# alexbuburuzan/MObI

Hardware: AMD Instinct MI355X
Metric: denoising throughput (UNet element-forwards/s = steps/s x UNet batch) (higher is better)
Workload: dtype bf16; 1 GPU; mobi_nusc_512 UNet denoising step, 8 objects/GPU (UNet batch 16), latent 64x64, DDIM-50 schedule, cfg_scale 1.0; objects_per_gpu=8, unet_batch=16, latent=64, sampler=ddim, parallelism=dp1 (objects sharded, no collective in the loop)

## Files before the change

### mobi_amd/csrc/igemm.hip

```cpp
#include <stdlib.h>

#include <type_traits>

#include "common.h"
#include "tuning.h"
#include "igemm_small.h"

#ifndef MOBI_FRAG2
#define MOBI_FRAG2 0
#endif
#ifndef MOBI_DMA_KS
#define MOBI_DMA_KS 1
#endif
#if defined(MOBI_IGEMM_FENCE) && MOBI_IGEMM_FENCE
#define MOBI_SCHED_FENCE() __builtin_amdgcn_sched_barrier(0)
#else
#define MOBI_SCHED_FENCE() ((void)0)
#endif

#ifndef MOBI_DBG_SKIP
#define MOBI_DBG_SKIP 0
#endif
#ifndef MOBI_PP_DMA_KS
#define MOBI_PP_DMA_KS 1
// ... 2515 lines not shown
    dim3 block(512);
    dim3 pgrid(grid.x < (unsigned)compute_units() ? grid.x : (unsigned)compute_units(), grid.y, grid.z);
    if (a.split_ws) {
      if (nt5) hipLaunchKernelGGL((igemm_pp_kernel<T, 5, false, true>), pgrid, block, 0, st, a);
      else     hipLaunchKernelGGL((igemm_pp_kernel<T, 4, false, true>), pgrid, block, 0, st, a);
    } else {
#define MOBI_PP_LAUNCH(NT_, G_) hipLaunchKernelGGL((igemm_pp_kernel<T, NT_, G_>), pgrid, block, 0, st, a)
      if (a.epilogue == MOBI_EPI_GEGLU) { if (nt5) MOBI_PP_LAUNCH(5, true); else MOBI_PP_LAUNCH(4, true); }
      else                              { if (nt5) MOBI_PP_LAUNCH(5, false); else MOBI_PP_LAUNCH(4, false); }
#undef MOBI_PP_LAUNCH
    }
  }
#ifdef MOBI_DEV
  else if (a.wm == 4 && a.fast && a.glds) {
    dim3 block(512);
    dim3 pgrid(grid.x < (unsigned)compute_units() ? grid.x : (unsigned)compute_units(), grid.y, grid.z);
    const int mode = tr ? 1 : (a.epi_direct ? (a.epilogue == MOBI_EPI_GEGLU ? 3 : 2) : 0);
#define MOBI_GLDS_LAUNCH(NT_, MODE_) hipLaunchKernelGGL((igemm_glds_kernel<T, NT_, MODE_>), pgrid, block, 0, st, a)
#define MOBI_GLDS_BY_MODE(NT_)                                                                     \
  do { switch (mode) { case 0: MOBI_GLDS_LAUNCH(NT_, 0); break; case 1: MOBI_GLDS_LAUNCH(NT_, 1); break; \
                       case 2: MOBI_GLDS_LAUNCH(NT_, 2); break; default: MOBI_GLDS_LAUNCH(NT_, 3); break; } } while (0)
    if (nt5) MOBI_GLDS_BY_MODE(5); else MOBI_GLDS_BY_MODE(4);
#undef MOBI_GLDS_BY_MODE
#undef MOBI_GLDS_LAUNCH
  }
#endif
  else if (a.wm == 4) { if (nt5) MOBI_IGEMM_BY_TR(5, 4); else MOBI_IGEMM_BY_TR(4, 4); }
  else if (a.sm && a.sm64) {
#define MOBI_SM64_LAUNCH_W(NT_, TR_, LNF_, OVL_) \
  hipLaunchKernelGGL((igemm_ring64_kernel<T, NT_, TR_, LNF_, OVL_>), grid, dim3(256), 0, st, a)
#define MOBI_SM64_LAUNCH(NT_, TR_, LNF_) \
  do { if (tuning().sm64_ovl != 0) MOBI_SM64_LAUNCH_W(NT_, TR_, LNF_, true); else MOBI_SM64_LAUNCH_W(NT_, TR_, LNF_, false); } while (0)
    if (a.ln_svec) { if (nt5) MOBI_SM64_LAUNCH(5, false, true); else MOBI_SM64_LAUNCH(4, false, true); }
    else if (nt5) { if (tr) MOBI_SM64_LAUNCH(5, true, false); else MOBI_SM64_LAUNCH(5, false, false); }
    else     { if (tr) MOBI_SM64_LAUNCH(4, true, false); else MOBI_SM64_LAUNCH(4, false, false); }
#undef MOBI_SM64_LAUNCH
#undef MOBI_SM64_LAUNCH_W
  }
  else if (a.sm) {
#define MOBI_SM_LAUNCH(NT_, TR_) hipLaunchKernelGGL((igemm_ring_kernel<T, NT_, TR_, 4, 4>), grid, dim3(256), 0, st, a)
    if (a.ln_svec) {
      if (nt5) hipLaunchKernelGGL((igemm_ring_kernel<T, 5, false, 4, 4, true>), grid, dim3(256), 0, st, a);
      else     hipLaunchKernelGGL((igemm_ring_kernel<T, 4, false, 4, 4, true>), grid, dim3(256), 0, st, a);
    }
    else if (nt5) { if (tr) MOBI_SM_LAUNCH(5, true); else MOBI_SM_LAUNCH(5, false); }
    else     { if (tr) MOBI_SM_LAUNCH(4, true); else MOBI_SM_LAUNCH(4, false); }
#undef MOBI_SM_LAUNCH
  }
  else                { if (nt5) MOBI_IGEMM_BY_TR(5, 2); else MOBI_IGEMM_BY_TR(4, 2); }
#undef MOBI_IGEMM_BY_TR
#undef MOBI_IGEMM_BY_FAST
#undef MOBI_IGEMM_LAUNCH
  MOBI_CHECK_LAUNCH();
  if (a.split_ws && !a.sync && !p->defer_finish) return launch_splitk_reduce<T>(a, st);
  return MOBI_OK;
}

constexpr int SMALL_MFLOP_DEFAULT = 1800, SMALL_MFLOP_K320 = 1000, SMALL_CONV_M_DEFAULT = 0;
static int small_tile(const mobi_igemm_params* p) {
  if (tuning().small == 0) return 0;
  if (tuning().small < 0 && (tuning().wm == 2 || tuning().wm == 4 || tuning().wide >= 0 || tuning().sm == 0)) return 0;
  const bool conv3 = p->kh == 3 && p->kw == 3 && p->pad_h == 1 && p->pad_w == 1;
  if (!(p->kh == 1 && p->kw == 1) && !conv3) return 0;
  if (p->stride != 1 || p->upsample || p->groups != 1 || p->epilogue != MOBI_EPI_NONE || p->k_order != 0 || p->split_k > 1) return 0;
  if (p->out_mode != MOBI_OUT_ROWS && p->out_mode != MOBI_OUT_ROWS_F32) return 0;
  if (p->hout != p->hin || p->wout != p->win) return 0;
  const int ct = p->c0 + p->c1, N = p->n_packed;
  const long long K = (long long)ct * p->kh * p->kw;
  if (ct % 320 || (p->c1 > 0 && p->c0 % 80) || N != p->cout || N % 32) return 0;
  const long long hw = (long long)p->hin * p->win, M = (long long)p->batch * hw;
  const long long ips = p->src_img_stride ? p->src_img_stride / p->c0 : hw;
  const long long cmax = p->c0 > p->c1 ? p->c0 : p->c1;
  if ((((long long)p->batch - 1) * ips + hw) * cmax * 2 >= 0x7fffffffLL || (long long)N * K * 2 >= 0x7fffffffLL) return 0;
  if (tuning().small > 0) return 32;
  if (conv3) {
    const int cap_m = tuning().small_conv_m >= 0 ? tuning().small_conv_m : SMALL_CONV_M_DEFAULT;
    return M <= cap_m ? 32 : 0;
  }
  const int cap = tuning().small_mflop >= 0 ? tuning().small_mflop : (K == 320 ? SMALL_MFLOP_K320 : SMALL_MFLOP_DEFAULT);
  if (2.0 * (double)M * N * (double)K > 1e6 * cap) return 0;
  return 32;
}

static int plan_splits(long long M, int n_packed, int ktot) {
  const int bn = (n_packed % 160) == 0 ? 160 : 128;
  const long long tiles = ((M + 127) / 128) * ((n_packed + bn - 1) / bn);
  const int nk = (ktot + 63) / 64;
  const bool r5 = tuning().split_round4 != 0;
  if (tiles >= 384 || nk < (r5 ? 24 : 16)) return 1;
  if (tiles >= 256 && (r5 ? nk <= 40 : nk < 40)) return 1;
  const long long target = tuning().split_target > 0 ? tuning().split_target : 512;
  long long s = (target + tiles - 1) / tiles;
  const long long cap = tiles <= 16 ? 16 : 8;
  if (s > cap) s = cap;
  if (s > nk / 8) s = nk / 8;
  if (r5) {
    if (s > 4 && s < 8) s = 4;
    if (s == 8 && nk <= 96 && tiles >= 64) s = 4;
  }
  if (tiles >= 128 && tiles <= 256 && s >= 2 && nk / s >= 80 && tuning().split_longk != 0) s *= 2;
  return s < 2 ? 1 : (int)s;
}

}

#if MOBI_STAMP
extern "C" int mobi_debug_set_stamps(void* buf) {
  return hipMemcpyToSymbol(HIP_SYMBOL(mobi::g_stamps), &buf, sizeof(void*)) == hipSuccess ? MOBI_OK : MOBI_ERR_LAUNCH;
}
#endif
#if MOBI_STAMP >= 2
extern "C" int mobi_debug_set_phases(void* buf) {
  return hipMemcpyToSymbol(HIP_SYMBOL(mobi::g_phase), &buf, sizeof(void*)) == hipSuccess ? MOBI_OK : MOBI_ERR_LAUNCH;
}
#endif

extern "C" int mobi_igemm_plan_splits(const mobi_igemm_params* p) {
  if (!p || p->groups != 1 || p->epilogue != MOBI_EPI_NONE || p->out_mode == MOBI_OUT_TRANSPOSED || p->ln_svec) return 1;
  {
    mobi_igemm_params q = *p;
    q.split_k = 0;
    if (mobi::small_tile(&q)) return 1;
  }
  return mobi::plan_splits((long long)p->batch * p->hout * p->wout, p->n_packed, p->kh * p->kw * (p->c0 + p->c1));
}

extern "C" size_t mobi_igemm_workspace_bytes(const mobi_igemm_params* p, int32_t splits) {
  if (!p || splits <= 1) return 0;
  return (size_t)splits * p->batch * p->hout * p->wout * p->n_packed * sizeof(float);
}

extern "C" size_t mobi_igemm_sync_bytes(const mobi_igemm_params* p, int32_t splits) {
  if (!p || splits <= 1) return 0;
  const size_t m = (size_t)p->batch * p->hout * p->wout;
  return ((m + 127) / 128) * (((size_t)p->n_packed + 127) / 128) * sizeof(int32_t);
}

static int igemm_prepare(const mobi_igemm_params* p, mobi::IgemmArgs& a) {
  using namespace mobi;
  if (!p || !p->src0 || !p->weight || !p->out) return MOBI_ERR_ARG;
  if (p->dtype != MOBI_F16 && p->dtype != MOBI_BF16) return MOBI_ERR_ARG;
  if (p->c0 <= 0 || (p->c0 & 31) || p->c1 < 0 || (p->c1 & 31) || (p->c1 > 0 && !p->src1)) return MOBI_ERR_UNSUPPORTED;
  if (p->batch <= 0 || p->hin <= 0 || p->win <= 0 || p->hout <= 0 || p->wout <= 0) return MOBI_ERR_ARG;
  if (p->kh <= 0 || p->kw <= 0 || p->stride <= 0 || p->groups <= 0 || p->batch % p->groups) return MOBI_ERR_ARG;
  if (p->cout <= 0 || p->n_packed <= 0) return MOBI_ERR_ARG;
  if (p->upsample != 0 && p->upsample != 1) return MOBI_ERR_ARG;
  const bool geglu = p->epilogue == MOBI_EPI_GEGLU;
  const bool leaky = p->epilogue == MOBI_EPI_LEAKY_RELU;
  if (p->epilogue != MOBI_EPI_NONE && !geglu && !leaky) return MOBI_ERR_ARG;
  if (leaky && (p->out_mode == MOBI_OUT_TRANSPOSED || p->ln_svec || p->split_k > 1 || p->k_order != 0))
    return MOBI_ERR_UNSUPPORTED;
  if (p->out_mode < 0 || p->out_mode > 2) return MOBI_ERR_ARG;
  if (p->out_mode != MOBI_OUT_TRANSPOSED && (p->cout & 7)) return MOBI_ERR_UNSUPPORTED;
  if (geglu && (p->out_mode != MOBI_OUT_ROWS || p->rowvec || p->residual)) return MOBI_ERR_UNSUPPORTED;
  if (!geglu && p->n_packed != p->cout) return MOBI_ERR_ARG;
  if (geglu && p->n_packed != 2 * p->cout) return MOBI_ERR_ARG;
  if (p->out_mode == MOBI_OUT_TRANSPOSED && (p->rowvec || p->residual)) return MOBI_ERR_UNSUPPORTED;
  if ((reinterpret_cast<uintptr_t>(p->bias) | reinterpret_cast<uintptr_t>(p->rowvec)) & 15) return MOBI_ERR_ALIGN;
  if (p->rowvec && (p->rowvec_stride & 3)) return MOBI_ERR_ALIGN;
  if ((reinterpret_cast<uintptr_t>(p->src0) | reinterpret_cast<uintptr_t>(p->src1) |
       reinterpret_cast<uintptr_t>(p->weight) | reinterpret_cast<uintptr_t>(p->out) |
       reinterpret_cast<uintptr_t>(p->residual)) & 15) return MOBI_ERR_ALIGN;

  const bool lnf = p->ln_svec != nullptr;
  if (lnf) {
    if (p->kh != 1 || p->kw != 1 || p->c1 || p->stride != 1 || p->upsample || p->groups != 1 || p->split_k > 1 || p->rowvec ||
        p->residual || p->out_mode == MOBI_OUT_TRANSPOSED || p->scale != 1.0f || p->k_order != 0 || p->hout != p->hin || p->wout != p->win)
      return MOBI_ERR_UNSUPPORTED;
    if (reinterpret_cast<uintptr_t>(p->ln_svec) & 15) return MOBI_ERR_ALIGN;
  }
  a.ln_svec = p->ln_svec; a.ln_eps = p->ln_eps;
  a.src0 = p->src0; a.src1 = p->src1;
  a.c0 = p->c0; a.c1 = p->c1; a.C = p->c0 + p->c1;
  a.hin = p->hin; a.win = p->win; a.up = p->upsample;
  a.hout = p->hout; a.wout = p->wout; a.hw_out = p->hout * p->wout;
  a.kh = p->kh; a.kw = p->kw; a.stride = p->stride; a.pad_h = p->pad_h; a.pad_w = p->pad_w;
  const long long hw_in = (long long)p->hin * p->win;
  if (p->src_img_stride && (p->c1 || p->src_img_stride % p->c0)) return MOBI_ERR_UNSUPPORTED;
  const long long ips = p->src_img_stride ? p->src_img_stride / p->c0 : hw_in;
  if (ips * p->batch > 0x7fffffffLL) return MOBI_ERR_UNSUPPORTED;
  a.img_pix_stride = (int)ips;
  a.weight = p->weight; a.w_group_stride = p->groups > 1 ? p->w_group_stride : 0;
  a.n_packed = p->n_packed; a.cout = p->cout;
  a.ktot = p->kh * p->kw * a.C;
  a.nk = (a.ktot + 63) / 64;
  a.imgs_per_group = p->batch / p->groups;
  a.M = a.imgs_per_group * a.hw_out;
  a.bias = p->bias; a.rowvec = p->rowvec; a.residual = p->residual;
  a.rowvec_stride = p->rowvec_stride ? p->rowvec_stride : p->cout;
  a.res_img_stride = p->res_img_stride ? p->res_img_stride : (long long)a.hw_out * p->cout;
  a.out = p->out;
  a.out_img_stride = p->out_img_stride ? p->out_img_stride : (long long)a.hw_out * p->cout;
  a.out_mode = p->out_mode; a.epilogue = p->epilogue; a.scale = p->scale;
  const int bn = (p->n_packed % 160) == 0 ? 160 : 128;
  {
    const long long tiles256 = ((a.M + 255) / 256) * (long long)((p->n_packed + bn - 1) / bn);
    a.wm = tiles256 >= 256 ? 4 : 2;
    if (p->split_k > 1 && a.M % 256 == 0 && tiles256 * p->split_k >= 256 && a.nk / p->split_k >= 16) a.wm = 4;
    if (tuning().pp_split == 0 && p->split_k > 1 && tiles256 < 256) a.wm = 2;
    if (tuning().wm == 2 || tuning().wm == 4) a.wm = tuning().wm;
  }
  a.tiles_m = (a.M + 64 * a.wm - 1) / (64 * a.wm);
  bool ring_ok = false;
  {
    const long long ext0 = (((long long)p->batch - 1) * ips + hw_in) * p->c0 * 2;
    const long long ext1 = p->c1 ? (((long long)p->batch - 1) * ips + hw_in) * p->c1 * 2 : 0;
    const long long wext = (long long)p->n_packed * a.ktot * 2;
// ... 185 lines not shown
```

### mobi_amd/ldm/modules/attention.py

```python
import os
import weakref

import torch
import torch.nn as nn

from ... import engine_dtype, ops
from ..._lib import ACT_NONE
from .diffusionmodules.util import Conv2d, GroupNorm32, LayerNorm, Linear, Marker, enter, leave, zero_module


FUSED_FF = os.environ.get("MOBI_FUSED_FF", "1") != "0"
FUSED_FF_MIN_ROWS = int(os.environ.get("MOBI_FUSED_FF_MIN_ROWS", "24576"))
FUSED_LN = os.environ.get("MOBI_FUSED_LN", "1") != "0"
ROW_CHAIN = os.environ.get("MOBI_ROW_CHAIN", "1") != "0"
LN_FOLD = os.environ.get("MOBI_LN_FOLD", "1") != "0"
LN_FOLD_MIN_ROWS = int(os.environ.get("MOBI_LN_FOLD_MIN_ROWS", "512"))
GROUPED_Q = os.environ.get("MOBI_GROUPED_Q", "1") != "0"
ROW_CHAIN_MIN_ROWS = int(os.environ.get("MOBI_ROW_CHAIN_MIN_ROWS", "24576"))
PRE_CHAIN = os.environ.get("MOBI_PRE_CHAIN", "0") == "1"


def _store_in_place(old, new):
    if isinstance(new, torch.Tensor):
        if isinstance(old, torch.Tensor) and old.shape == new.shape and old.dtype == new.dtype \
                and old.device == new.device and old.is_contiguous() and old.data_ptr() != new.data_ptr():
            old.copy_(new)
            return old
        return new.contiguous()
    if isinstance(new, tuple):
        if not (isinstance(old, tuple) and len(old) == len(new)):
            old = (None,) * len(new)
        return tuple(_store_in_place(o, n) for o, n in zip(old, new))
    return new


def Normalize(in_channels):
    return GroupNorm32(32, in_channels, eps=1e-6)


class GEGLU(nn.Module):
    def __init__(self, dim_in, dim_out):
        super().__init__()
        self.proj = Linear(dim_in, dim_out * 2)

    def forward(self, x, ln=None):
        if ln is None:
            return ops.linear(x, self.proj.packed_geglu())
        ps = (self.proj.weight, self.proj.bias, ln.weight, ln.bias)
        key = tuple(p._version for p in ps) + (ps[0].data_ptr(), ps[0].device, engine_dtype(), ln.eps)
        c = self.__dict__.setdefault("_ln_cache", {})
        if c.get("key") != key:
            w, b = ops.fold_layernorm(self.proj.weight, self.proj.bias, ln.weight, ln.bias)
            c["key"], c["val"] = key, ops.with_row_sums(ops.pack_geglu(w, b, engine_dtype(), self.proj.weight.device), ln.eps)
        return ops.linear(x, c["val"])


class FeedForward(nn.Module):
    def __init__(self, dim, dim_out=None, mult=4, glu=False, dropout=0.):
        super().__init__()
        if not glu:
            raise NotImplementedError("MObI's transformer blocks use gated_ff=True")
        inner_dim = int(dim * mult)
        dim_out = dim if dim_out is None else dim_out
        self.net = nn.Sequential(GEGLU(dim, inner_dim), Marker(), Linear(inner_dim, dim_out))

    def _fused(self):
        proj, out = self.net[0].proj, self.net[2]
        c, hidden = out.weight.shape
        if not (FUSED_FF and ops.ff_geglu_supported(c, hidden) and proj.weight.shape == (2 * hidden, c)):
            return None
        ps = (proj.weight, proj.bias, out.weight, out.bias)
        key = tuple(p._version for p in ps) + (ps[0].data_ptr(), ps[0].device, engine_dtype())
        cache = self.__dict__.setdefault("_fused_cache", {})
        if cache.get("key") != key:
            cache["key"], cache["val"] = key, ops.pack_ff_geglu(proj.weight, proj.bias, out.weight, out.bias, engine_dtype(),
                                                                proj.weight.device)
        return cache["val"]

    def forward(self, x, residual=None, norm=None):
        rows = x.numel() // x.shape[-1]
        pf = self._fused() if (rows >= FUSED_FF_MIN_ROWS and x.is_contiguous()
                               and (residual is None or residual.is_contiguous())) else None
        if pf is not None:
            if norm is not None and FUSED_LN:
                return ops.ff_geglu(x, pf, residual=residual, ln=(*norm.affine(), norm.eps))
            if norm is not None:
                x = ops.layernorm(x, *norm.affine(), norm.eps)
            return ops.ff_geglu(x, pf, residual=residual)
        if norm is not None and LN_FOLD and x.is_contiguous() and rows >= LN_FOLD_MIN_ROWS:
            return ops.linear(self.net[0](x, ln=norm), self.net[2].packed(), residual=residual)
        if norm is not None:
            x = ops.layernorm(x, *norm.affine(), norm.eps)
        return ops.linear(self.net[0](x), self.net[2].packed(), residual=residual)


class CrossAttention(nn.Module):
    def __init__(self, query_dim, context_dim=None, heads=8, dim_head=64, dropout=0.):
        super().__init__()
        inner_dim = dim_head * heads
        context_dim = query_dim if context_dim is None else context_dim
        self.scale = dim_head ** -0.5
        self.heads = heads
        self.inner_dim = inner_dim
        self.to_q = Linear(query_dim, inner_dim, bias=False)
        self.to_k = Linear(context_dim, inner_dim, bias=False)
        self.to_v = Linear(context_dim, inner_dim, bias=False)
        self.to_out = nn.Sequential(Linear(inner_dim, query_dim), Marker())

    def _stacked(self, names, fold_q=False, ln=None):
        mods = [getattr(self, n) for n in names]
        dtype = engine_dtype()
        key = (names, fold_q, dtype, self.scale) + tuple(v for m in mods for v in (m.weight._version, m.weight.data_ptr()))
        if ln is not None:
            key += (ln.weight._version, ln.bias._version, ln.weight.data_ptr(), ln.eps)
        c = self.__dict__.setdefault("_stack_cache", {})
        slot = (names, fold_q, ln is not None)
        hit = c.get(slot)
        if hit is None or hit[0] != key:
            ws = [m.weight.detach() for m in mods]
            if fold_q:
                assert names[0] == "to_q"
                ws[0] = ws[0].float() * (self.scale * ops.LOG2E)
            w = torch.cat([w_.float() for w_ in ws], dim=0) if (fold_q or ln is not None) else torch.cat(ws, dim=0)
            if ln is not None:
                wf, bf = ops.fold_layernorm(w, None, ln.weight, ln.bias)
                hit = (key, ops.with_row_sums(ops.pack_linear(wf, bf, dtype, w.device), ln.eps))
            else:
                hit = (key, ops.pack_linear(w, None, dtype, w.device))
            c[slot] = hit
        return hit[1]

    def self_attention(self, xn, ln=None):
        c = self.inner_dim
        qkv = ops.linear(xn, self._stacked(("to_q", "to_k", "to_v"), fold_q=True, ln=ln))
        return ops.attention(qkv[..., :c], qkv[..., c:2 * c], qkv[..., 2 * c:], self.heads, self.scale, v_rows=True,
                             q_log2_scaled=True)

    def token_attention(self, xn, ctx, q=None):
        c = self.inner_dim
        if q is not None:
            kv = ops.linear(ctx, self._stacked(("to_k", "to_v")))
        else:
            q, kv = ops.concurrently(lambda: ops.linear(xn, self._stacked(("to_q",), fold_q=True)),
                                     lambda: ops.linear(ctx, self._stacked(("to_k", "to_v"))))
        return ops.attention(q, kv[..., :c], kv[..., c:], self.heads, self.scale, v_rows=True, q_log2_scaled=True)

    def context_kv(self, context):
        n, tk, cc = context.shape
        flat = context.reshape(n * tk, cc)
        wk, _ = self.to_k.skinny()
        wv, _ = self.to_v.skinny()
        k = ops.skinny_linear(flat, wk).reshape(n, tk, self.inner_dim)
        v = ops.skinny_linear(flat, wv).reshape(n, tk, self.inner_dim)
        return k, v

    def few_token_attention(self, xn, context):
        q, (k, v) = ops.concurrently(lambda: ops.linear(xn, self.to_q.packed()), lambda: self.context_kv(context))
        return ops.ctx_attention(q, k, v, self.heads, self.scale)

    def single_token_vector(self, token, extra_bias=None):
        wv, _ = self.to_v.skinny()
        wo, bo = self.to_out[0].skinny()
        if extra_bias is not None:
            bo = bo + extra_bias.detach().float()
        return ops.skinny_linear(ops.skinny_linear(token, wv), wo, bo)

    def attend(self, x, context=None, q=None):
        if context is None:
            return self.self_attention(x)
        if context.dtype == torch.float32:
            if context.shape[1] > 8:
                raise NotImplementedError("fp32 contexts with more than 8 tokens")
            return self.few_token_attention(x, context.contiguous())
        return self.token_attention(x, context, q=q)

    def forward(self, x, context=None, mask=None):
# ... 32 lines not shown
        self.norm2 = LayerNorm(dim)
        self.norm3 = LayerNorm(dim)
        if bbox_cond:
            self.cond_adapter_norm = LayerNorm(dim)
            self.cond_adapter_connector = zero_module(Linear(dim, dim))
        if multimodal:
            self.cross_modal_norm_camera = LayerNorm(dim)
            self.cross_modal_connector_camera = zero_module(Linear(dim, dim))
            self.cross_modal_norm_lidar = LayerNorm(dim)
            self.cross_modal_connector_lidar = zero_module(Linear(dim, dim))
        self.checkpoint = checkpoint

    def _folded(self, attn, connector, tag):
        lo, lc = attn.to_out[0], connector
        key = (tag, lo.weight._version, lo.bias._version, lc.weight._version, lc.bias._version,
               lo.weight.data_ptr(), lo.packed().w.dtype)
        cache = self.__dict__.setdefault("_fold_cache", {})
        hit = cache.get(tag)
        if hit is None or hit[0] != key:
            wc, wo = lc.weight.detach().double().cpu(), lo.weight.detach().double().cpu()
            w = (wc @ wo).float()
            b = (wc @ lo.bias.detach().double().cpu() + lc.bias.detach().double().cpu()).float()
            hit = (key, ops.pack_linear(w, b, lo.packed().w.dtype, lo.weight.device))
            cache[tag] = hit
        return hit[1]

    @staticmethod
    def _ln(norm, x):
        g, b = norm.affine()
        return ops.layernorm(x, g, b, norm.eps)

    def _cross_modal_queries(self, ln_cam, ln_lidar):
        cam, lid = self.cross_modal_attn_camera, self.cross_modal_attn_lidar
        if not (GROUPED_Q and ln_cam is not None and ln_lidar is not None and ln_cam.shape == ln_lidar.shape
                and ln_cam.is_contiguous() and ln_lidar.is_contiguous() and cam.inner_dim == lid.inner_dim
                and ln_lidar.data_ptr() == ln_cam.data_ptr() + ln_cam.numel() * ln_cam.element_size()):
            return None, None
        dtype = engine_dtype()
        ws = (cam.to_q.weight, lid.to_q.weight)
        key = (dtype, cam.scale, lid.scale) + tuple(v for w in ws for v in (w._version, w.data_ptr()))
        c = self.__dict__.setdefault("_q_pair_cache", {})
        if c.get("key") != key:
            w = torch.cat([cam.to_q.weight.detach().float() * (cam.scale * ops.LOG2E),
                           lid.to_q.weight.detach().float() * (lid.scale * ops.LOG2E)], dim=0)
            c["key"], c["val"] = key, ops.pack_linear(w, None, dtype, w.device)
        h, t, ch = ln_cam.shape
        both = ln_cam.as_strided((2 * h, t, ch), (t * ch, ch, 1))
        q = ops.linear(both, c["val"], groups=2)
        return q[:h], q[h:]

    def _chain_weights(self):
        a1, cam, lid = self.attn1, self.cross_modal_attn_camera, self.cross_modal_attn_lidar
        nc, nl = self.cross_modal_norm_camera, self.cross_modal_norm_lidar
        cc, cl = self.cross_modal_connector_camera, self.cross_modal_connector_lidar
        ps = [a1.to_out[0].weight, cam.to_q.weight, cam.to_k.weight, cam.to_v.weight, cam.to_out[0].weight, cam.to_out[0].bias,
              lid.to_q.weight, lid.to_k.weight, lid.to_v.weight, lid.to_out[0].weight, lid.to_out[0].bias,
              nc.weight, nc.bias, nl.weight, nl.bias, cc.weight, cc.bias, cl.weight, cl.bias]
        dtype = engine_dtype()
        key = tuple(p._version for p in ps) + (ps[0].data_ptr(), ps[0].device, dtype)
        c = self.__dict__.setdefault("_chain_cache", {})
        if c.get("key") != key:
            dev = ps[0].device
            pk = lambda w, b=None, **kw: ops.pack_chain_weight(w, b, dtype, dev, **kw)

            def fold(attn, con):
                wc, wo = con.weight.detach().double().cpu(), attn.to_out[0].weight.detach().double().cpu()
                return pk((wc @ wo).float(), (wc @ attn.to_out[0].bias.detach().double().cpu() + con.bias.detach().double().cpu()).float())

            c["key"] = key
            c["val"] = {"to_out": pk(a1.to_out[0].weight),
                        "q_cam": pk(cam.to_q.weight, ln=(nc.weight, nc.bias), scale=cam.scale * ops.LOG2E),
                        "q_lid": pk(lid.to_q.weight, ln=(nl.weight, nl.bias), scale=lid.scale * ops.LOG2E),
                        "k_cam": pk(cam.to_k.weight), "v_cam": pk(cam.to_v.weight),
                        "k_lid": pk(lid.to_k.weight), "v_lid": pk(lid.to_v.weight),
                        "fold_cam": fold(cam, cc), "fold_lid": fold(lid, cl)}
        return c["val"]

    def _chain_ok(self, x, adapter, adapter_image):
        return (ROW_CHAIN and self.bbox_cond and adapter is not None and adapter_image is not None and self.multimodal
                and x.shape[0] % 2 == 0
                and x.is_contiguous() and x.shape[0] * x.shape[1] >= ROW_CHAIN_MIN_ROWS
                and ops.row_chain_supported(x.shape[2], x.shape[1]))

    def _forward_chained(self, x, a, ref_vec, adapter_image):
        n, t, c = x.shape
        cw = self._chain_weights()
        cam, lid = self.cross_modal_attn_camera, self.cross_modal_attn_lidar
        nc, nl = self.cross_modal_norm_camera, self.cross_modal_norm_lidar
        new = lambda *shape: torch.empty(shape, device=x.device, dtype=x.dtype)
        q_cam, q_lid, kv_l, kv_c = new(n // 2, t, c), new(n // 2, t, c), new(n // 2, t, 2 * c), new(n // 2, t, 2 * c)
        x_in, x = x, new(n, t, c)

        def head(prog):
            return prog.load(a, "s").load(x_in, "r").product(cw["to_out"], resid=True, to_s=True, bias=ref_vec,
                                                             bias_img_stride=c).adapter(dst=x)
        p_cam = head(ops.ChainProgram()).rowstats(nc.eps).product(cw["q_cam"], fold=True, dst=q_cam, dst_img_div=2)
        p_lid = head(ops.ChainProgram()).rowstats(nl.eps).product(cw["q_lid"], fold=True, dst=q_lid, dst_img_div=2)
        p_lid.product(cw["k_cam"], dst=kv_l[..., :c], dst_img_div=2).product(cw["v_cam"], dst=kv_l[..., c:], dst_img_div=2)
        rows = n * t
        ops.row_chain([p_cam, p_lid], n, t, x.dtype, adapter=(adapter_image, self.cond_adapter_norm.eps),
                      flops=2.0 * rows * c * c * 3.5, nbytes=2.0 * rows * c * 5.0, note=f"post_attn1 rows={rows}")
        xc, xl = x[::2], x[1::2]
        ac = ops.attention(q_cam, kv_l[..., :c], kv_l[..., c:], cam.heads, cam.scale, v_rows=True, q_log2_scaled=True)
        p = ops.ChainProgram().load(ac, "s").load(xc, "r").product(cw["fold_cam"], resid=True, to_s=True, dst=xc)
        p.product(cw["k_lid"], dst=kv_c[..., :c]).product(cw["v_lid"], dst=kv_c[..., c:])
        ops.row_chain([p], n // 2, t, x.dtype, flops=2.0 * (rows // 2) * c * c * 3, nbytes=2.0 * (rows // 2) * c * 5.0,
                      note=f"post_cam rows={rows // 2}")
        al = ops.attention(q_lid, kv_c[..., :c], kv_c[..., c:], lid.heads, lid.scale, v_rows=True, q_log2_scaled=True)
        ops.linear(al, self._folded(lid, self.cross_modal_connector_lidar, "lidar"), residual=xl, out=xl)
        return self.ff(x, residual=x, norm=self.norm3)

    def forward(self, x, context=None, qkv=None):
        return self._forward(x, context, qkv=qkv)

    def _context_terms(self, ctx):
        ws = [self.attn2.to_v.weight, self.attn2.to_out[0].weight, self.attn2.to_out[0].bias, self.attn1.to_out[0].bias]
        if self.bbox_cond:
            ca = self.cond_adapter_attn
            ws += [ca.to_k.weight, ca.to_v.weight, ca.to_q.weight, ca.to_out[0].weight, ca.to_out[0].bias,
                   self.cond_adapter_connector.weight, self.cond_adapter_connector.bias,
                   self.cond_adapter_norm.weight, self.cond_adapter_norm.bias]
        key = (ctx._version, ctx.data_ptr(), tuple(ctx.shape), tuple(w._version for w in ws),
               ws[0].data_ptr(), self.attn2.to_v.skinny()[0].dtype)
        slots = self.__dict__.setdefault("_ctx_slots", {})
        sid = id(ctx)
        c = slots.get(sid)
        if c is None or c["ref"]() is not ctx:
            c = {"ref": weakref.ref(ctx, lambda _r, s_=slots, i_=sid: s_.pop(i_, None)), "key": None}
            slots[sid] = c
        if c["key"] != key:
            c["key"] = key
            ref_vec = self.attn2.single_token_vector(ctx[:, 0], extra_bias=self.attn1.to_out[0].bias)
            kv = self.cond_adapter_attn.context_kv(ctx) if self.bbox_cond else None
            adapter = self._two_key_terms(kv) if self.bbox_cond and ctx.shape[1] == 2 else None
            image = None
            if adapter is not None and ROW_CHAIN and self.cond_adapter_attn.heads <= 8 and ops.row_chain_supported(adapter[0].shape[2], 128):
                image = ops.chain_adapter_image(adapter[0], adapter[2], adapter[3], adapter[4], engine_dtype())
            for name, val in (("ref_vec", ref_vec), ("kv", kv), ("adapter", adapter), ("adapter_image", image)):
                c[name] = _store_in_place(c.get(name), val)
        return c["ref_vec"], c["kv"], c["adapter"], c["adapter_image"]

    def context_term_addresses(self, ctx):
        c = self.__dict__.get("_ctx_slots", {}).get(id(ctx))
        if c is None or c["ref"]() is not ctx or c["key"] is None:
            return None
        flat = []
        for name in ("ref_vec", "kv", "adapter", "adapter_image"):
            v = c.get(name)
            for t in (v if isinstance(v, tuple) else (v,)):
                flat.append(None if t is None else t.data_ptr())
        return tuple(flat)

    def _two_key_params(self):
        ca, ln, con = self.cond_adapter_attn, self.cond_adapter_norm, self.cond_adapter_connector
        ps = [ca.to_q.weight, ca.to_out[0].weight, ca.to_out[0].bias, con.weight, con.bias, ln.weight, ln.bias]
        key = tuple(p._version for p in ps) + (ps[0].data_ptr(), ps[0].device)
        c = self.__dict__.setdefault("_two_key_cache", {})
        if c.get("key") != key:
            d = lambda t: t.detach().double().cpu()
            wq, wo, bo, wc, bc, gamma, beta = (d(p) for p in ps)
            h, inner = ca.heads, wq.shape[0]
            mask = torch.zeros(h, inner, dtype=torch.float64)
            for i in range(h):
                mask[i, i * (inner // h):(i + 1) * (inner // h)] = 1.0
            f = lambda t: t.float().contiguous().to(ps[0].device)
            c["key"], c["val"] = key, (f(wc @ wo), f(wc @ bo + bc), f(wq.t()), f(gamma * ca.scale), f(beta * ca.scale), f(mask))
        return c["val"]

    def _two_key_terms(self, kv):
        w, b0, wqt, gamma_s, beta_s, mask = self._two_key_params()
        k, v = kv[0].float(), kv[1].float()
        n, _, inner = k.shape
        h = self.cond_adapter_attn.heads
        dk = ((k[:, 0] - k[:, 1])[:, None, :] * mask[None]).reshape(n * h, inner).contiguous()
        dv = ((v[:, 0] - v[:, 1])[:, None, :] * mask[None]).reshape(n * h, inner).contiguous()
        wt = ops.linear_f32(dk, wqt).view(n, h, -1)
        a = (wt * gamma_s).contiguous()
        c = (wt * beta_s).sum(-1).contiguous()
        u = ops.linear_f32(dv, w).view(n, h, -1).contiguous()
        b = ops.linear_f32(v[:, 1].contiguous(), w, b0)
        return a, a.sum(-1).contiguous(), c, u, b

    def _forward(self, x, context=None, qkv=None):
        ctx = context.float().contiguous()
        ref_vec, ctx_kv, adapter, adapter_image = self._context_terms(ctx)
        if qkv is not None:
            c = self.attn1.inner_dim
            a = ops.attention(qkv[..., :c], qkv[..., c:2 * c], qkv[..., 2 * c:], self.attn1.heads, self.attn1.scale, v_rows=True,
                              q_log2_scaled=True)
        elif LN_FOLD and x.is_contiguous() and x.shape[0] * x.shape[1] >= LN_FOLD_MIN_ROWS:
            a = self.attn1.self_attention(x, ln=self.norm1)
        else:
            a = self.attn1.self_attention(self._ln(self.norm1, x))
        if self._chain_ok(x, adapter, adapter_image):
            return self._forward_chained(x, a, ref_vec, adapter_image)
        x = ops.linear(a, self.attn1.to_out[0].packed(), residual=x, rowvec=ref_vec, rowvec_has_bias=True)

        ln_cam = ln_lidar = None
        if self.bbox_cond and adapter is not None:
            nc, nl = (self.cross_modal_norm_camera, self.cross_modal_norm_lidar) if self.multimodal else (None, None)
            if (FUSED_LN and self.multimodal and x.shape[0] % 2 == 0 and nc.eps == nl.eps
                    and ops.two_key_adapter_fuses_ln(x.shape[2], x.shape[0] * x.shape[1])):
                x, (ln_cam, ln_lidar) = ops.two_key_adapter(x, *adapter, eps=self.cond_adapter_norm.eps, out=x,
                                                            ln_pair=(nc.affine(), nl.affine(), nc.eps))
            else:
                x = ops.two_key_adapter(x, *adapter, eps=self.cond_adapter_norm.eps, out=x)
        elif self.bbox_cond:
            ca = self.cond_adapter_attn
            q = ops.linear(self._ln(self.cond_adapter_norm, x), ca.to_q.packed())
            a = ops.ctx_attention(q, ctx_kv[0], ctx_kv[1], ca.heads, ca.scale)
            x = ops.linear(a, self._folded(self.cond_adapter_attn, self.cond_adapter_connector, "adapter"),
                           residual=x)

        if self.multimodal:
            if x.shape[0] % 2:
                raise ValueError("multimodal blocks need camera/lidar samples interleaved on an even batch")
            xc, xl = x[::2], x[1::2]
            q_cam, q_lid = self._cross_modal_queries(ln_cam, ln_lidar)
            a = self.cross_modal_attn_camera.attend(self._ln(self.cross_modal_norm_camera, xc) if ln_cam is None else ln_cam,
                                                    context=xl, q=q_cam)
            ops.linear(a, self._folded(self.cross_modal_attn_camera, self.cross_modal_connector_camera, "cam"),
                       residual=xc, out=xc)
            a = self.cross_modal_attn_lidar.attend(self._ln(self.cross_modal_norm_lidar, xl) if ln_lidar is None else ln_lidar,
                                                   context=xc, q=q_lid)
            ops.linear(a, self._folded(self.cross_modal_attn_lidar, self.cross_modal_connector_lidar, "lidar"),
                       residual=xl, out=xl)

        return self.ff(x, residual=x, norm=self.norm3)


class SpatialTransformer(nn.Module):
    def __init__(self, in_channels, n_heads, d_head, depth=1, dropout=0., context_dim=None, bbox_cond=False,
                 multimodal=False):
        super().__init__()
        self.in_channels = in_channels
        inner_dim = n_heads * d_head
        self.norm = Normalize(in_channels)
        self.proj_in = Conv2d(in_channels, inner_dim, kernel_size=1, stride=1, padding=0)
        self.transformer_blocks = nn.ModuleList(
            [BasicTransformerBlock(inner_dim, n_heads, d_head, dropout=dropout, context_dim=context_dim,
                                   bbox_cond=bbox_cond, multimodal=multimodal) for _ in range(depth)])
        self.proj_out = zero_module(Conv2d(inner_dim, in_channels, kernel_size=1, stride=1, padding=0))

    def _pre_weights(self):
        blk = self.transformer_blocks[0]
        a1, n1 = blk.attn1, blk.norm1
        ps = [self.proj_in.weight, self.proj_in.bias, a1.to_q.weight, a1.to_k.weight, a1.to_v.weight, n1.weight, n1.bias]
        dtype = engine_dtype()
        key = tuple(p._version for p in ps) + (ps[0].data_ptr(), ps[0].device, dtype)
        c = self.__dict__.setdefault("_pre_cache", {})
        if c.get("key") != key:
            dev = ps[0].device
            pk = lambda w, b=None, **kw: ops.pack_chain_weight(w, b, dtype, dev, **kw)
            ln = (n1.weight, n1.bias)
            c["key"] = key
            c["val"] = {"proj_in": pk(self.proj_in.weight[:, :, 0, 0], self.proj_in.bias),
                        "q": pk(a1.to_q.weight, ln=ln, scale=a1.scale * ops.LOG2E), "k": pk(a1.to_k.weight, ln=ln),
                        "v": pk(a1.to_v.weight, ln=ln)}
        return c["val"]

    def _pre_chain_ok(self, x):
        n, h, w, c = x.shape
        return (ROW_CHAIN and PRE_CHAIN and len(self.transformer_blocks) == 1 and c == self.proj_in.weight.shape[0] and x.is_contiguous()
                and n * h * w >= ROW_CHAIN_MIN_ROWS and ops.row_chain_supported(c, h * w) and c % 64 == 0)

    def forward(self, x, context=None):
        x, ext = enter(x)
        n, h, w, c = x.shape
        g, b = self.norm.affine()
        if isinstance(x, ops.Deferred) and self._pre_chain_ok(x.tensor):
            x = x.finish()
        if not isinstance(x, ops.Deferred) and self._pre_chain_ok(x):
            blk = self.transformer_blocks[0]
            cw = self._pre_weights()
            scale, shift = ops.groupnorm_scale_shift(x, g, b, self.norm.eps)
            t = torch.empty((n, h * w, c), device=x.device, dtype=x.dtype)
            qkv = torch.empty((n, h * w, 3 * c), device=x.device, dtype=x.dtype)
            prog = ops.ChainProgram().load(x.view(n, h * w, c), "s").affine(scale, shift).product(cw["proj_in"], to_s=True, dst=t)
            prog.rowstats(blk.norm1.eps).product(cw["q"], fold=True, dst=qkv[..., :c]).product(cw["k"], fold=True, dst=qkv[..., c:2 * c])
            prog.product(cw["v"], fold=True, dst=qkv[..., 2 * c:])
            rows = n * h * w
            ops.row_chain([prog], n, h * w, x.dtype, flops=2.0 * rows * c * c * 4, nbytes=2.0 * rows * c * 5.0, note=f"pre_attn1 rows={rows}")
            t = blk(t, context=context, qkv=qkv)
            y = ops.igemm(t.view(n, h, w, t.shape[2]), self.proj_out.packed(), residual=x)
            return leave(y, ext)
        xn = ops.groupnorm(x, g, b, self.norm.eps, silu=False)
        x = ops.finished(x)
        t = ops.igemm(xn, self.proj_in.packed())
        t = t.view(n, h * w, t.shape[3])
        for block in self.transformer_blocks:
            t = block(t, context=context)
        y = ops.igemm(t.view(n, h, w, t.shape[2]), self.proj_out.packed(), residual=x)
        return leave(y, ext)
```

### mobi_amd/ldm/modules/diffusionmodules/openaimodel.py

```python
import torch
import torch.nn as nn

from .... import engine_dtype, ops
from ...._lib import ACT_SILU
from ..attention import SpatialTransformer
from .util import (Conv2d, Marker, conv_nd, enter, leave, linear, normalization, timestep_embedding, zero_module)


class TimestepBlock(nn.Module):
    pass


def _opens_with_groupnorm(layer):
    if isinstance(layer, nn.Sequential):
        return len(layer) > 0 and _opens_with_groupnorm(layer[0])
    return isinstance(layer, (ResBlock, SpatialTransformer))


class TimestepEmbedSequential(nn.Sequential, TimestepBlock):
    def forward(self, x, emb, context=None, skip=None, then_groupnorm=False):
        layers = list(self)
        for i, layer in enumerate(layers):
            defer = _opens_with_groupnorm(layers[i + 1]) if i + 1 < len(layers) else then_groupnorm
            if isinstance(layer, TimestepBlock):
                x = layer(x, emb, skip=skip, defer_out=defer)
                skip = None
            elif isinstance(layer, SpatialTransformer):
                x = layer(x, context)
            elif isinstance(layer, Conv2d):
                x = _plain_conv(layer, ops.finished(x))
            elif isinstance(layer, (Upsample, Downsample)):
                x = layer(x, defer_out=defer)
            else:
                x = layer(ops.finished(x))
        return x


def _plain_conv(conv, x):
    if isinstance(x, (list, tuple)) or (x.dtype == torch.float32 and conv.in_channels <= 16):
        srcs = list(x) if isinstance(x, (list, tuple)) else [x]
        packed = ops.pack_sources([s.float().contiguous() for s in srcs], engine_dtype())
        return ops.igemm(packed, conv.packed_thin(), stride=conv.stride, pad=conv.padding)
    x, ext = enter(x)
    return leave(ops.igemm(x, conv.packed(), stride=conv.stride, pad=conv.padding), ext)


class Upsample(nn.Module):
    def __init__(self, channels, use_conv, dims=2, out_channels=None, padding=1):
        super().__init__()
        assert use_conv and dims == 2, "MObI uses conv_resample=True, dims=2"
        self.channels = channels
        self.out_channels = out_channels or channels
        self.conv = conv_nd(dims, self.channels, self.out_channels, 3, padding=padding)

    def forward(self, x, defer_out=False):
        x, ext = enter(ops.finished(x))
        assert x.shape[3] == self.channels
        defer = "keep" if defer_out and not ext else None
        return leave(ops.igemm(x, self.conv.packed(), upsample=True, pad=self.conv.padding, defer=defer), ext)


class Downsample(nn.Module):
    def __init__(self, channels, use_conv, dims=2, out_channels=None, padding=1):
        super().__init__()
        assert use_conv and dims == 2, "MObI uses conv_resample=True, dims=2"
        self.channels = channels
        self.out_channels = out_channels or channels
        self.op = conv_nd(dims, self.channels, self.out_channels, 3, stride=2, padding=padding)

    def forward(self, x, defer_out=False):
        x, ext = enter(ops.finished(x))
        assert x.shape[3] == self.channels
        defer = "keep" if defer_out and not ext else None
        return leave(ops.igemm(x, self.op.packed(), stride=2, pad=self.op.padding, defer=defer), ext)


class ResBlock(TimestepBlock):
    def __init__(self, channels, emb_channels, dropout, out_channels=None, use_conv=False,
                 use_scale_shift_norm=False, dims=2, use_checkpoint=False, up=False, down=False):
        super().__init__()
        if use_scale_shift_norm or up or down or use_conv:
            raise NotImplementedError("not used by MObI's UNet configuration")
        self.channels = channels
        self.emb_channels = emb_channels
        self.out_channels = out_channels or channels
        self.in_layers = nn.Sequential(normalization(channels), Marker(),
                                       conv_nd(dims, channels, self.out_channels, 3, padding=1))
        self.emb_layers = nn.Sequential(Marker(), linear(emb_channels, self.out_channels))
        self.out_layers = nn.Sequential(normalization(self.out_channels), Marker(), Marker(),
                                        zero_module(conv_nd(dims, self.out_channels, self.out_channels, 3, padding=1)))
        if self.out_channels == channels:
            self.skip_connection = Marker()
        else:
            self.skip_connection = conv_nd(dims, channels, self.out_channels, 1)
        self._emb_slice = None

    def forward(self, x, emb, skip=None, defer_out=False):
        x, ext = enter(x)
        if skip is not None:
            skip, _ = enter(ops.finished(skip))
        if isinstance(emb, dict):
            lo, hi = self._emb_slice
            emb_out = emb["proj"][:, lo:hi]
        else:
            w, b = self.emb_layers[1].skinny()
            emb_out = ops.skinny_linear(emb.float().contiguous(), w, b + self.in_layers[2].bias.detach().float(),
                                        pre_act=ACT_SILU)
        n1, n2 = self.in_layers[0], self.out_layers[0]

        g, b = n1.affine()
        h1 = ops.groupnorm(x, g, b, n1.eps, silu=True, x2=skip)
# ... 140 lines not shown
```

### mobi_amd/ops.py

```python
import ctypes as C
import math
import os
from dataclasses import dataclass
from typing import Optional

import torch

from . import _lib
from ._lib import (ACT_GELU, ACT_NONE, ACT_SILU, EPI_GEGLU, EPI_LEAKY_RELU, EPI_NONE, MOBI_BF16, MOBI_F16, OUT_ROWS, OUT_ROWS_F32,
                   OUT_TRANSPOSED)


_PROFILE = None


def set_profiler(sink):
    global _PROFILE
    _PROFILE = sink


_HEALTH = None


def set_health(sink):
# ... 783 lines not shown
        self.tiles = torch.from_numpy(tmap.view(np.uint8)).to(self.device)


def repack_multi(table):
    _lib.check(_lib.load().mobi_repack_multi(_ptr(table.entries), table.count, _ptr(table.tiles), table.n_tiles, _dt(table.dtype),
                                             _stream()), "mobi_repack_multi")


def geglu_fwd(pre):
    lib = _lib.load()
    assert pre.is_contiguous()
    inner = pre.shape[-1] // 2
    h = torch.empty(pre.shape[:-1] + (inner,), device=pre.device, dtype=pre.dtype)
    _lib.check(lib.mobi_geglu_fwd(_ptr(pre), _ptr(h), pre.numel() // (2 * inner), inner, _dt(pre.dtype), _stream()), "mobi_geglu_fwd")
    return h


def geglu_bwd(pre, dh):
    lib = _lib.load()
    assert pre.is_contiguous() and dh.is_contiguous()
    inner = pre.shape[-1] // 2
    dpre = torch.empty_like(pre)
    _lib.check(lib.mobi_geglu_bwd(_ptr(pre), _ptr(dh), _ptr(dpre), pre.numel() // (2 * inner), inner, _dt(pre.dtype), _stream()),
               "mobi_geglu_bwd")
    return dpre


def attention_bwd(q, k, v, o, dout, heads, scale, force_vector=False):
    lib = _lib.load()
    n, tq, tk = q.shape[0], q.shape[1], k.shape[1]
    c = o.shape[2]
    new = lambda t_: torch.empty((n, t_, c), device=q.device, dtype=q.dtype)
    dq, dk, dv = new(tq), new(tk), new(tk)
    lse = torch.empty((2, n, heads, tq), device=q.device, dtype=torch.float32)
    p = _lib.AttentionBwdParams()
    for name, t_ in (("q", q), ("k", k), ("v", v), ("o", o), ("dout", dout)):
        assert t_.shape[2] == 1 or t_.stride(2) == 1
        setattr(p, name, _ptr(t_))
        setattr(p, name + "_img_stride", t_.stride(0))
        setattr(p, name + "_row_stride", t_.stride(1))
    p.dq, p.dk, p.dv, p.lse, p.dvec = _ptr(dq), _ptr(dk), _ptr(dv), _ptr(lse[0]), _ptr(lse[1])
    p.images, p.heads, p.dh, p.tq, p.tk, p.scale, p.dtype = n, heads, c // heads, tq, tk, scale, _dt(q.dtype)
    p.force_vector = int(force_vector)
    _lib.check(lib.mobi_attention_bwd(C.byref(p), _stream()), "mobi_attention_bwd")
    return dq, dk, dv


FUSED_SPLIT = os.environ.get("MOBI_FUSED_SPLIT", "0") == "1"
_SYNC = {}


def _sync_counters(device, nbytes):
    key = (device, torch.cuda.current_stream(device).cuda_stream)
    buf = _SYNC.get(key)
    if buf is None or buf.numel() * 4 < nbytes:
        buf = torch.zeros((max(nbytes // 4 + 1, 1 << 16),), device=device, dtype=torch.int32)
        _SYNC[key] = buf
    return buf


DEFER_SPLIT = os.environ.get("MOBI_DEFER_SPLIT", "1") != "0"


class Deferred:

    def __init__(self, tensor, params, ws, refs, keep):
        self.tensor, self.params, self.ws, self.refs, self.keep = tensor, params, ws, refs, keep
        self.label = None if _HEALTH is None else _HEALTH.label()
        self.count = _lib.load().mobi_igemm_slab_count(C.byref(params))
        assert self.count >= 2, self.count
        self.done = False

    @property
    def shape(self):
        return self.tensor.shape

    @property
    def dtype(self):
        return self.tensor.dtype

    @property
    def device(self):
        return self.tensor.device

    def finish(self):
        if not self.done:
            m = self.tensor.numel() // self.tensor.shape[3]
            with _Timed("split_finish", 0.0, self.count * m * self.params.n_packed * 4.0 + self.tensor.numel() * 2.0,
                        f"m={m} n={self.params.n_packed} slabs={self.count}"):
                _lib.check(_lib.load().mobi_igemm_finish(C.byref(self.params), _stream()), "mobi_igemm_finish")
            self._release()
            if _HEALTH is not None:
                _HEALTH.measure("split_finish", self.tensor, label=self.label)
        return self.tensor

    def _release(self):
        self.done = True
        self.ws = self.refs = None


def finished(x):
    return x.finish() if isinstance(x, Deferred) else x


def igemm(x, pw: Packed, *, x2=None, stride=1, pad=None, upsample=False, hout=None, wout=None, rowvec=None,
          rowvec_has_bias=False, residual=None, out=None, out_mode=OUT_ROWS, scale=1.0, weight_per_image=False,
          w_group_stride=0, split_k=None, groups=1, defer=None, leaky=False):
    lib = _lib.load()
    x, x2, residual = finished(x), finished(x2), finished(residual)
    n, hin, win, c0 = x.shape
    c1 = 0 if x2 is None else x2.shape[3]
    assert c0 + c1 == pw.cin, (c0, c1, pw.cin)
    if groups > 1:
        assert not weight_per_image and not pw.geglu and pw.bias is None and n % groups == 0 and pw.cout % groups == 0
        pw = Packed(pw.w, None, pw.kh, pw.kw, pw.cin, pw.cout // groups, pw.n_packed // groups, wt=pw.wt)
        w_group_stride = pw.n_packed * pw.kh * pw.kw * pw.cin
    ph, pw_ = (pw.kh // 2, pw.kw // 2) if pad is None else pad
    hl, wl = (hin * 2, win * 2) if upsample else (hin, win)
    if hout is None:
        hout = (hl + 2 * ph - pw.kh) // stride + 1
        wout = (wl + 2 * pw_ - pw.kw) // stride + 1
    if out is None:
        if out_mode == OUT_TRANSPOSED:
            out = torch.empty((n, pw.cout, hout * wout), device=x.device, dtype=x.dtype)
        elif out_mode == OUT_ROWS_F32:
            out = torch.empty((n, hout, wout, pw.cout), device=x.device, dtype=torch.float32)
        else:
            out = torch.empty((n, hout, wout, pw.cout), device=x.device, dtype=x.dtype)
    p = _lib.IgemmParams()
    p.src0, p.src1 = _ptr(x), _ptr(x2)
    p.c0, p.c1, p.batch, p.hin, p.win = c0, c1, n, hin, win
    p.upsample, p.hout, p.wout = int(upsample), hout, wout
    p.kh, p.kw, p.stride, p.pad_h, p.pad_w = pw.kh, pw.kw, stride, ph, pw_
    dense_in = hin * win * c0
    s = _img_stride(x)
    p.src_img_stride = 0 if s == dense_in else s
    p.weight = _ptr(pw.w)
    p.weight_tiled = None if weight_per_image else _ptr(pw.wt)
    p.groups = n if weight_per_image else groups
    p.w_group_stride = w_group_stride
    p.n_packed, p.cout = pw.n_packed, pw.cout
    assert rowvec is not None or not rowvec_has_bias
    p.bias, p.rowvec, p.residual = (None if rowvec_has_bias else _ptr(pw.bias)), _ptr(rowvec), _ptr(residual)
    if rowvec is not None:
        assert rowvec.dtype == torch.float32 and rowvec.stride(1) == 1 and rowvec.shape == (n, pw.cout)
        p.rowvec_stride = rowvec.stride(0)
    dense_out = hout * wout * pw.cout
    if residual is not None:
        s = _img_stride(residual)
        p.res_img_stride = 0 if s == dense_out else s
    s = _img_stride(out)
    p.out = _ptr(out)
    p.out_img_stride = 0 if s == dense_out else s
    p.out_mode = out_mode
    assert not (leaky and pw.geglu)
    p.epilogue = EPI_GEGLU if pw.geglu else (EPI_LEAKY_RELU if leaky else EPI_NONE)
    p.scale = scale
    p.k_order = pw.k_order
    if pw.svec is not None:
        assert pw.svec.dtype == torch.float32 and pw.svec.numel() == pw.n_packed and pw.bias is not None and not rowvec_has_bias
        p.ln_svec, p.ln_eps = _ptr(pw.svec), pw.ln_eps
        split_k = 1
    if pw.k_order and (c0 % 64 or (c1 and c1 % 64)):
        raise ValueError("chunk-major weights need 64-channel-aligned sources")
    p.dtype = _dt(x.dtype)
    splits = split_k if split_k is not None else lib.mobi_igemm_plan_splits(C.byref(p))
# ... 914 lines not shown
```

Before: 816.0 UNet element-forwards/s.

## Fold transformer proj_out into FF output linear and allow deferred split-k finish

Algebraically folds the SpatialTransformer proj_out 1x1 conv into the feed-forward output linear, precomputing in float64 on the host a concatenated weight [Wpo·W2, Wpo] and bias, applied as one igemm over the FF hidden plus the residual stream. This removes one GEMM and the intermediate write/read of the transformer output, at the cost of a wider K dimension and possible bf16 rounding differences from the folded weights. It also lets the transformer output defer split-k finishing to a following groupnorm consumer, and slightly tweaks split-k planning thresholds for pointwise convs.

```diff
diff --git a/mobi_amd/csrc/igemm.hip b/mobi_amd/csrc/igemm.hip
--- a/mobi_amd/csrc/igemm.hip
+++ b/mobi_amd/csrc/igemm.hip
@@ -2621,12 +2621,12 @@
   return 32;
 }
 
-static int plan_splits(long long M, int n_packed, int ktot) {
+static int plan_splits(long long M, int n_packed, int ktot, bool pointwise) {
   const int bn = (n_packed % 160) == 0 ? 160 : 128;
   const long long tiles = ((M + 127) / 128) * ((n_packed + bn - 1) / bn);
   const int nk = (ktot + 63) / 64;
   const bool r5 = tuning().split_round4 != 0;
-  if (tiles >= 384 || nk < (r5 ? 24 : 16)) return 1;
+  if (tiles >= 384 || nk < (r5 ? (pointwise ? 26 : 24) : 16)) return 1;
   if (tiles >= 256 && (r5 ? nk <= 40 : nk < 40)) return 1;
   const long long target = tuning().split_target > 0 ? tuning().split_target : 512;
   long long s = (target + tiles - 1) / tiles;
@@ -2635,7 +2635,7 @@
   if (s > nk / 8) s = nk / 8;
   if (r5) {
     if (s > 4 && s < 8) s = 4;
-    if (s == 8 && nk <= 96 && tiles >= 64) s = 4;
+    if (s == 8 && nk <= 100 && tiles >= 64) s = 4;
   }
   if (tiles >= 128 && tiles <= 256 && s >= 2 && nk / s >= 80 && tuning().split_longk != 0) s *= 2;
   return s < 2 ? 1 : (int)s;
@@ -2661,7 +2661,8 @@
     q.split_k = 0;
     if (mobi::small_tile(&q)) return 1;
   }
-  return mobi::plan_splits((long long)p->batch * p->hout * p->wout, p->n_packed, p->kh * p->kw * (p->c0 + p->c1));
+  return mobi::plan_splits((long long)p->batch * p->hout * p->wout, p->n_packed, p->kh * p->kw * (p->c0 + p->c1),
+                           p->kh * p->kw == 1);
 }
 
 extern "C" size_t mobi_igemm_workspace_bytes(const mobi_igemm_params* p, int32_t splits) {
diff --git a/mobi_amd/ldm/modules/attention.py b/mobi_amd/ldm/modules/attention.py
--- a/mobi_amd/ldm/modules/attention.py
+++ b/mobi_amd/ldm/modules/attention.py
@@ -18,6 +18,7 @@
 GROUPED_Q = os.environ.get("MOBI_GROUPED_Q", "1") != "0"
 ROW_CHAIN_MIN_ROWS = int(os.environ.get("MOBI_ROW_CHAIN_MIN_ROWS", "24576"))
 PRE_CHAIN = os.environ.get("MOBI_PRE_CHAIN", "0") == "1"
+PROJ_FOLD = os.environ.get("MOBI_PROJ_FOLD", "1") != "0"
 
 
 def _store_in_place(old, new):
@@ -34,6 +35,29 @@
     return new
 
 
+def fold_proj_out(w2, b2, wpo, bpo):
+    d = lambda t: t.detach().double().cpu()
+    w2, b2, wpo, bpo = d(w2), d(b2), d(wpo), d(bpo)
+    wpo = wpo.reshape(wpo.shape[0], -1)
+    return torch.cat([wpo @ w2, wpo], dim=1), wpo @ b2 + bpo
+
+
+def fold_is_finite(w, b, dtype):
+    return bool(torch.isfinite(w.to(dtype)).all()) and bool(torch.isfinite(b.to(dtype)).all())
+
+
+class ProjTail:
+
+    def __init__(self, owner, x_in, defer=None, tape=None):
+        self.owner, self.proj_out, self.x_in, self.defer, self.tape = owner, owner.proj_out, x_in, defer, tape
+        self.out = None
+
+    @staticmethod
+    def allowed(depth, tape=None, tensors=()):
+        return (PROJ_FOLD and depth == 1 and tape is None
+                and all(t.is_contiguous() and not t.requires_grad for t in tensors))
+
+
 def Normalize(in_channels):
     return GroupNorm32(32, in_channels, eps=1e-6)
 
@@ -77,7 +101,22 @@
                                                                 proj.weight.device)
         return cache["val"]
 
-    def forward(self, x, residual=None, norm=None):
+    def proj_fold_key(self, proj_out):
+        ps = (self.net[2].weight, self.net[2].bias, proj_out.weight, proj_out.bias)
+        return tuple(p._version for p in ps) + (ps[0].data_ptr(), ps[0].device, engine_dtype())
+
+    def _proj_fold(self, proj_out):
+        key = self.proj_fold_key(proj_out)
+        cache = self.__dict__.setdefault("_proj_fold_cache", {})
+        if cache.get("key") != key:
+            out = self.net[2]
+            w, b = fold_proj_out(out.weight, out.bias, proj_out.weight, proj_out.bias)
+            ok = fold_is_finite(w, b, engine_dtype())
+            cache["key"] = key
+            cache["val"] = ops.pack_linear(w.float(), b.float(), engine_dtype(), out.weight.device) if ok else None
+        return cache["val"]
+
+    def forward(self, x, residual=None, norm=None, tail=None):
         rows = x.numel() // x.shape[-1]
         pf = self._fused() if (rows >= FUSED_FF_MIN_ROWS and x.is_contiguous()
                                and (residual is None or residual.is_contiguous())) else None
@@ -87,11 +126,21 @@
             if norm is not None:
                 x = ops.layernorm(x, *norm.affine(), norm.eps)
             return ops.ff_geglu(x, pf, residual=residual)
+        pf = None
+        if (tail is not None and residual is x and tail.proj_out.weight.shape[1] == self.net[2].weight.shape[0]
+                and ProjTail.allowed(1, tail.tape, (x, tail.x_in))):
+            pf = self._proj_fold(tail.proj_out)
         if norm is not None and LN_FOLD and x.is_contiguous() and rows >= LN_FOLD_MIN_ROWS:
-            return ops.linear(self.net[0](x, ln=norm), self.net[2].packed(), residual=residual)
-        if norm is not None:
-            x = ops.layernorm(x, *norm.affine(), norm.eps)
-        return ops.linear(self.net[0](x), self.net[2].packed(), residual=residual)
+            hid = self.net[0](x, ln=norm)
+        else:
+            hid = self.net[0](x if norm is None else ops.layernorm(x, *norm.affine(), norm.eps))
+        if pf is None:
+            return ops.linear(hid, self.net[2].packed(), residual=residual)
+        n, h, w, c = tail.x_in.shape
+        with ops.health_scope(tail.owner):
+            y = ops.igemm(hid.unsqueeze(2), pf, x2=x.unsqueeze(2), residual=tail.x_in.view(n, h * w, 1, c), defer=tail.defer)
+        tail.out = y.view(n, h, w, pf.cout)
+        return None
 
 
 class CrossAttention(nn.Module):
@@ -290,7 +339,7 @@
                 and x.is_contiguous() and x.shape[0] * x.shape[1] >= ROW_CHAIN_MIN_ROWS
                 and ops.row_chain_supported(x.shape[2], x.shape[1]))
 
-    def _forward_chained(self, x, a, ref_vec, adapter_image):
+    def _forward_chained(self, x, a, ref_vec, adapter_image, tail=None):
         n, t, c = x.shape
         cw = self._chain_weights()
         cam, lid = self.cross_modal_attn_camera, self.cross_modal_attn_lidar
@@ -316,10 +365,10 @@
                       note=f"post_cam rows={rows // 2}")
         al = ops.attention(q_lid, kv_c[..., :c], kv_c[..., c:], lid.heads, lid.scale, v_rows=True, q_log2_scaled=True)
         ops.linear(al, self._folded(lid, self.cross_modal_connector_lidar, "lidar"), residual=xl, out=xl)
-        return self.ff(x, residual=x, norm=self.norm3)
-
-    def forward(self, x, context=None, qkv=None):
-        return self._forward(x, context, qkv=qkv)
+        return self.ff(x, residual=x, norm=self.norm3, tail=tail)
+
+    def forward(self, x, context=None, qkv=None, tail=None):
+        return self._forward(x, context, qkv=qkv, tail=tail)
 
     def _context_terms(self, ctx):
         ws = [self.attn2.to_v.weight, self.attn2.to_out[0].weight, self.attn2.to_out[0].bias, self.attn1.to_out[0].bias]
@@ -389,7 +438,7 @@
         b = ops.linear_f32(v[:, 1].contiguous(), w, b0)
         return a, a.sum(-1).contiguous(), c, u, b
 
-    def _forward(self, x, context=None, qkv=None):
+    def _forward(self, x, context=None, qkv=None, tail=None):
         ctx = context.float().contiguous()
         ref_vec, ctx_kv, adapter, adapter_image = self._context_terms(ctx)
         if qkv is not None:
@@ -401,7 +450,7 @@
         else:
             a = self.attn1.self_attention(self._ln(self.norm1, x))
         if self._chain_ok(x, adapter, adapter_image):
-            return self._forward_chained(x, a, ref_vec, adapter_image)
+            return self._forward_chained(x, a, ref_vec, adapter_image, tail=tail)
         x = ops.linear(a, self.attn1.to_out[0].packed(), residual=x, rowvec=ref_vec, rowvec_has_bias=True)
 
         ln_cam = ln_lidar = None
@@ -434,7 +483,7 @@
             ops.linear(a, self._folded(self.cross_modal_attn_lidar, self.cross_modal_connector_lidar, "lidar"),
                        residual=xl, out=xl)
 
-        return self.ff(x, residual=x, norm=self.norm3)
+        return self.ff(x, residual=x, norm=self.norm3, tail=tail)
 
 
 class SpatialTransformer(nn.Module):
@@ -472,10 +521,20 @@
         return (ROW_CHAIN and PRE_CHAIN and len(self.transformer_blocks) == 1 and c == self.proj_in.weight.shape[0] and x.is_contiguous()
                 and n * h * w >= ROW_CHAIN_MIN_ROWS and ops.row_chain_supported(c, h * w) and c % 64 == 0)
 
-    def forward(self, x, context=None):
+    def _tail(self, x, defer):
+        return ProjTail(self, x, defer) if ProjTail.allowed(len(self.transformer_blocks), None, (x,)) else None
+
+    def _proj_out(self, t, x, tail):
+        if tail is not None and tail.out is not None:
+            return tail.out
+        n, h, w, _ = x.shape
+        return ops.igemm(t.view(n, h, w, t.shape[2]), self.proj_out.packed(), residual=x)
+
+    def forward(self, x, context=None, defer_out=False):
         x, ext = enter(x)
         n, h, w, c = x.shape
         g, b = self.norm.affine()
+        defer = "keep" if defer_out and not ext else None
         if isinstance(x, ops.Deferred) and self._pre_chain_ok(x.tensor):
             x = x.finish()
         if not isinstance(x, ops.Deferred) and self._pre_chain_ok(x):
@@ -489,14 +548,14 @@
             prog.product(cw["v"], fold=True, dst=qkv[..., 2 * c:])
             rows = n * h * w
             ops.row_chain([prog], n, h * w, x.dtype, flops=2.0 * rows * c * c * 4, nbytes=2.0 * rows * c * 5.0, note=f"pre_attn1 rows={rows}")
-            t = blk(t, context=context, qkv=qkv)
-            y = ops.igemm(t.view(n, h, w, t.shape[2]), self.proj_out.packed(), residual=x)
-            return leave(y, ext)
+            tail = self._tail(x, defer)
+            t = blk(t, context=context, qkv=qkv, tail=tail)
+            return leave(self._proj_out(t, x, tail), ext)
         xn = ops.groupnorm(x, g, b, self.norm.eps, silu=False)
         x = ops.finished(x)
         t = ops.igemm(xn, self.proj_in.packed())
         t = t.view(n, h * w, t.shape[3])
+        tail = self._tail(x, defer)
         for block in self.transformer_blocks:
-            t = block(t, context=context)
-        y = ops.igemm(t.view(n, h, w, t.shape[2]), self.proj_out.packed(), residual=x)
-        return leave(y, ext)
+            t = block(t, context=context, tail=tail)
+        return leave(self._proj_out(t, x, tail), ext)
diff --git a/mobi_amd/ldm/modules/diffusionmodules/openaimodel.py b/mobi_amd/ldm/modules/diffusionmodules/openaimodel.py
--- a/mobi_amd/ldm/modules/diffusionmodules/openaimodel.py
+++ b/mobi_amd/ldm/modules/diffusionmodules/openaimodel.py
@@ -26,7 +26,7 @@
                 x = layer(x, emb, skip=skip, defer_out=defer)
                 skip = None
             elif isinstance(layer, SpatialTransformer):
-                x = layer(x, context)
+                x = layer(x, context, defer_out=defer)
             elif isinstance(layer, Conv2d):
                 x = _plain_conv(layer, ops.finished(x))
             elif isinstance(layer, (Upsample, Downsample)):
diff --git a/mobi_amd/ops.py b/mobi_amd/ops.py
--- a/mobi_amd/ops.py
+++ b/mobi_amd/ops.py
@@ -889,6 +889,11 @@
     @property
     def device(self):
         return self.tensor.device
+
+    def view(self, *shape):
+        assert len(shape) == 4 and shape[0] == self.tensor.shape[0] and shape[3] == self.tensor.shape[3]
+        self.tensor = self.tensor.view(*shape)
+        return self
 
     def finish(self):
         if not self.done:
```

Result: no change. 822.5 UNet element-forwards/s (median of 6 runs) (+0.8%).
